# kernel-matrix-benchmarks/kernel-matrix-benchmarks

Measured on AMD Instinct MI355X. Metric: point-pair interactions/s (N*M/s) + max |err| vs scipy, D=3 Gaussian, higher is better.
Workload: dtype f32

## Files before the change

kernel_matrix_benchmarks_amd/csrc/kmvp_api.hip:

```cpp
#include "kmvp_ctx.hpp"

namespace kmvp {

Rccl g_rccl;

namespace {
thread_local std::string g_create_error;
}

int fail(kmvp_ctx* c, int code, const std::string& msg) {
  if (c) c->err = msg;
  else g_create_error = msg;
  return code;
}
const char* create_error() { return g_create_error.c_str(); }

int ensure(kmvp_ctx* c, DevBuf& b, size_t bytes) {
  if (bytes <= b.cap && b.p) return KMVP_OK;
  if (b.p) {
    HIP_TRY(c, hipFree(b.p));
    b.p = nullptr;
    b.cap = 0;
  }
  if (bytes == 0) bytes = 16;
// ... 284 lines not shown
    g_rccl.CommDestroy(c->comm);
    c->comm = nullptr;
  }
  c->host_xchg = fn;
  c->host_user = user;
  c->comm_count = world;
  c->rank = rank;
  c->world = world;
  return KMVP_OK;
}

int kmvp_comm_world(const kmvp_ctx* c) { return (c && c->exchanges()) ? c->comm_count : 1; }
int kmvp_comm_rank(const kmvp_ctx* c) { return (c && c->exchanges()) ? c->rank : 0; }

int kmvp_set_option(kmvp_ctx* c, const char* key, int64_t value) {
  if (!c || !key) return KMVP_E_INVALID;
  const std::string k(key);
  if (k == "feed") {
    if (value < -1 || value > 1) return fail(c, KMVP_E_INVALID, "feed must be -1 (auto), 0 or 1");
    c->opt_feed = (int)value;
  } else if (k == "targets_per_lane") {
    if (value != 0 && value != 1 && value != 2 && value != 4 && value != 8)
      return fail(c, KMVP_E_INVALID, "targets_per_lane must be 0 (auto), 1, 2, 4 or 8");
    c->opt_T = (int)value;
  } else if (k == "segments") {
    if (value < 0 || value > 65535) return fail(c, KMVP_E_INVALID, "segments out of range");
    c->opt_segments = (int)value;
  } else if (k == "fast_sqdists") {
    if (value < -1 || value > 4) return fail(c, KMVP_E_INVALID, "fast_sqdists must be -1 (auto), 0, 1, 2, 3 or 4");
    c->opt_fast = (int)value;
  } else if (k == "cellmm_shape") {
    if (value < -1 || value > 1) return fail(c, KMVP_E_INVALID, "cellmm_shape must be -1 (by size), 0 (32x32x16) or 1 (16x16x32)");
    c->opt_cellmm_shape = (int)value;
  } else if (k == "cell_fused") {
    if (value < -1 || value > 1) return fail(c, KMVP_E_INVALID, "cell_fused must be -1 (automatic), 0 (two launches) or 1 (one launch where it applies)");
    c->opt_cell_fused = (int)value;
  } else if (k == "mfma_variant") {
    if (value != -1 && value != 0 && value != 1 && value != 4 && value != 5)
      return fail(c, KMVP_E_INVALID, "mfma_variant must be -1 (by kernel), 0, 1, 4 or 5");
    c->opt_mfma_variant = (int)value;
  } else if (k == "same_points_global") {
    c->opt_same_global = value != 0;
  } else if (k == "partial_shard") {
    c->opt_partial = value != 0;
  } else if (k == "fast_tiles") {
    if (value != 0 && value != 1 && value != 2 && value != 4 && value != 8)
      return fail(c, KMVP_E_INVALID, "fast_tiles must be 0 (auto), 1, 2, 4 or 8");
    c->opt_fast_tiles = (int)value;
  } else if (k == "chunk") {
    if (value < 8 || value > (1 << 24)) return fail(c, KMVP_E_INVALID, "chunk out of range");
    c->opt_chunk = (int)value;
  } else {
    return fail(c, KMVP_E_INVALID, "unknown option " + k);
  }
  return KMVP_OK;
}

int64_t kmvp_device_bytes(const kmvp_ctx* c) {
  if (!c) return 0;
  size_t t = 0;
  for (const DevBuf* b : {&c->y_raw, &c->x_raw, &c->b_raw, &c->xs, &c->rec, &c->x_scaled,
                          &c->y_scaled, &c->part, &c->partd, &c->aux, &c->sortbuf, &c->perm, &c->sums, &c->out, &c->scratch, &c->sdiag, &c->xchg, &c->kexp, &c->kshift, &c->xchgk, &c->kflag,
                    &c->sk_xs_x, &c->sk_rec_y, &c->sk_xs_y, &c->sk_rec_x, &c->sk_state,
                          &c->cell_tperm, &c->cell_sperm, &c->cell_tgrp, &c->cell_sgrp, &c->cell_slot, &c->cell_tmeta, &c->cell_sums, &c->cell_skey, &c->cell_scentre, &c->cell_scale})
    t += b->cap;
  return (int64_t)t;
// ... 9 lines not shown
```

kernel_matrix_benchmarks_amd/csrc/kmvp_cellmm.hpp:

```cpp
#pragma once
#include <hip/hip_runtime.h>
#include <stdint.h>

#include "kmvp_cell.hpp"

namespace kmvp {

#ifndef CMM_BF16
#define CMM_BF16 0
#endif
#if CMM_BF16
typedef __bf16 cmm_half;
#else
typedef _Float16 cmm_half;
#endif
typedef cmm_half f16x8 __attribute__((ext_vector_type(8)));
typedef cmm_half f16x2 __attribute__((ext_vector_type(2)));

constexpr int CMM_STAGE_TILES = 12;
constexpr int CMM_STAGE_BYTES = 8192;
constexpr int CMM_E_OFF = 0;
constexpr int CMM_B_OFF = CMM_STAGE_TILES * CELL_TILE * 16;
constexpr int CMM_HDR_OFF = CMM_B_OFF + CMM_STAGE_TILES * CELL_TILE * 4;
static_assert(CMM_HDR_OFF + CMM_STAGE_TILES * 16 <= CMM_STAGE_BYTES, "stage image too small");
// ... 229 lines not shown
        acc[tt] = __builtin_amdgcn_mfma_f32_32x32x16_f16(ya, xb[tt], acc[tt], 0, 0, 0);
#endif
      }
    }
    if (s + 1 < s_end) commit(buf ^ 1);
    __syncthreads();
  }
  if (key_s >= 0) fold();

  const double inv = (double)a.scale[1];
#pragma unroll
  for (int tt = 0; tt < TT; ++tt)
    if (h == 0) a.part[(int64_t)seg * a.n_slots + (tile0 + tt - a.tile_base) * CELL_TILE + r] = outd[tt] * inv;
}


__device__ __forceinline__ float cellmm16_fold4(float a, float b, float c, float d) {
  const auto p = __builtin_amdgcn_permlane16_swap(__float_as_uint(a), __float_as_uint(b), false, false);
  const float w0 = __uint_as_float(p[0]) + __uint_as_float(p[1]);
  const auto q = __builtin_amdgcn_permlane16_swap(__float_as_uint(c), __float_as_uint(d), false, false);
  const float w1 = __uint_as_float(q[0]) + __uint_as_float(q[1]);
  const auto r = __builtin_amdgcn_permlane32_swap(__float_as_uint(w0), __float_as_uint(w1), false, false);
  return __uint_as_float(r[0]) + __uint_as_float(r[1]);
}
__device__ __forceinline__ float cellmm16_sources_sum(float v) {
  v += cellmm_dpp<0x111, 0xf>(v);
  v += cellmm_dpp<0x112, 0xf>(v);
  v += cellmm_dpp<0x114, 0xf>(v);
  v += cellmm_dpp<0x118, 0xf>(v);
  return __int_as_float(__builtin_amdgcn_readlane(__float_as_int(v), 15)) +
         __int_as_float(__builtin_amdgcn_readlane(__float_as_int(v), 47));
}

#ifndef CMM16_NOFOLD
#define CMM16_NOFOLD 0
#endif

template <int TT>
__device__ __forceinline__ void cellmm16_body(const CellmmArgs& a, int bid, unsigned char (*lds)[CMM_STAGE_BYTES]) {
  static_assert(!CMM_BF16, "f16 operands only");
  constexpr int SB = CMM_STAGE_BYTES;
  constexpr int PIECES = SB / (16 * BLOCK_THREADS);
  constexpr float LOG2E = 1.4426950408889634f;
  constexpr int HT = 2 * TT;
  constexpr int NG = (HT + 3) / 4;

  int tb, seg;
  block_to_work(bid, a.segments, a.tile_blocks, tb, seg);
  const int lane = threadIdx.x & 63;
  const int wave = threadIdx.x >> 6;
  const int cc = lane & 15;
  const int kg = lane >> 4;
  const int h = kg & 1;
  const int rs = 16 * (kg >> 1) + cc;
  const int64_t tile0 = a.tile_base + ((int64_t)tb * WAVES_PER_BLOCK + wave) * TT;

  float cT[3];
  f16x8 xb[HT];
#pragma unroll
  for (int u = 0; u < HT; ++u) {
    const f32x4 v = *reinterpret_cast<const f32x4*>(a.xd + ((tile0 + (u >> 1)) * CELL_TILE + 16 * (u & 1) + cc) * 4);
    xb[u] = cellmm_target_operand(v, h);
  }
  {
    const f32x4 m = *reinterpret_cast<const f32x4*>(a.tmeta + tile0 * 4);
#pragma unroll
    for (int c = 0; c < 3; ++c) cT[c] = __int_as_float(__builtin_amdgcn_readfirstlane(__float_as_int(m[c])));
  }
// ... 11 lines not shown
  }

  f32x4 acc[HT];
#pragma unroll
  for (int u = 0; u < HT; ++u)
#pragma unroll
    for (int k = 0; k < 4; ++k) acc[u][k] = 0.f;

  const int64_t s_begin = (int64_t)seg * a.seg_stages;
  int64_t s_end = s_begin + a.seg_stages;
  if (s_end > a.m_stages) s_end = a.m_stages;

  f32x4 pre[PIECES];
  auto fetch = [&](int64_t s) {
    const unsigned char* src = a.img + s * SB;
#pragma unroll
    for (int p = 0; p < PIECES; ++p)
      pre[p] = *reinterpret_cast<const f32x4*>(src + (p * BLOCK_THREADS + (int)threadIdx.x) * 16);
  };
  auto commit = [&](int buf) {
#pragma unroll
    for (int p = 0; p < PIECES; ++p)
      *reinterpret_cast<f32x4*>(&lds[buf][(p * BLOCK_THREADS + (int)threadIdx.x) * 16]) = pre[p];
  };
  if (s_begin < s_end) {
    fetch(s_begin);
    commit(0);
  }
  __syncthreads();

  int key_s = -2;
  float S0 = 0.f, S0c = 0.f;
  float D1[3] = {0.f, 0.f, 0.f};

  auto fold = [&]() {
#if CMM16_NOFOLD
    asm volatile("" ::"v"(S0), "v"(S0c));
#else
    const float s0 = cellmm16_sources_sum(S0) * CMM_TARGET_SCALE;
    float x[4 * NG];
#pragma unroll
    for (int u = 0; u < 4 * NG; ++u) x[u] = u < HT ? (acc[u][0] + acc[u][1]) + (acc[u][2] + acc[u][3]) : 0.f;
#pragma unroll
    for (int g = 0; g < NG; ++g) {
      const float v = cellmm16_fold4(x[4 * g], x[4 * g + 1], x[4 * g + 2], x[4 * g + 3]);
      outd[g] += (double)(U[g] * ((v - vprev[g]) + s0));
      vprev[g] = v;
    }
#endif
    S0 = 0.f;
    S0c = 0.f;
  };
  auto new_cell = [&](const f32x4 cs, int ks) {
    if (key_s >= 0) fold();
    key_s = ks;
#pragma unroll
    for (int c = 0; c < 3; ++c) D1[c] = (cT[c] - cs[c]) * LOG2E;
#if !CMM16_NOFOLD
#pragma unroll
    for (int g = 0; g < NG; ++g) {
      float s2 = 0.f;
#pragma unroll
      for (int c = 0; c < 3; ++c) {
        const float df = dl[g][c] + (cT[c] - cs[c]);
        s2 = fmaf(df, df, s2);
      }
      U[g] = kexp2(s2 * -LOG2E);
    }
#endif
  };

  for (int64_t s = s_begin; s < s_end; ++s) {
    const int buf = (int)((s - s_begin) & 1);
    if (s + 1 < s_end) fetch(s + 1);
    const unsigned char* base = &lds[buf][0];
    const unsigned char* p_ef = base + CMM_E_OFF + rs * 16;
    const unsigned char* p_b = base + CMM_B_OFF + rs * 4;
    const f32x4* hdr = reinterpret_cast<const f32x4*>(base + CMM_HDR_OFF);
    const int keys = lane < CMM_STAGE_TILES ? __float_as_int(hdr[lane < CMM_STAGE_TILES ? lane : 0][3]) : -1;
#pragma unroll 1
    for (int q = 0; q < CMM_STAGE_TILES; ++q) {
      const int ks = __builtin_amdgcn_readlane(keys, q);
      if (ks < 0) break;
      if (ks != key_s) new_cell(hdr[q], ks);
      const f32x4 ef = *reinterpret_cast<const f32x4*>(p_ef);
      const float bq = *reinterpret_cast<const float*>(p_b);
      p_ef += CELL_TILE * 16;
      p_b += CELL_TILE * 4;
      const float m0 = h ? ef[2] : ef[0];
      const float m1 = h ? ef[0] : ef[1];
      const float m2 = h ? ef[2] : 1.f;
      const f32x4 a14 = f32x4{m0, m1 * m2, m0 * m0, m1 * ef[1]};
      const float a5 = ef[1] * m2;
      const float arg = fmaf(ef[0], D1[0], fmaf(ef[1], D1[1], fmaf(ef[2], D1[2], ef[3])));
      const float wb = kexp2(arg) * bq;
      {
        const float yk = wb - S0c;
        const float tk = S0 + yk;
        S0c = (tk - S0) - yk;
        S0 = tk;
      }
      const float u1 = a14[0] * wb, u2 = a14[1] * wb;
      const f16x2 R0 = cellmm_pk(u1, u2);
      const float c1 = (float)R0[0], c2 = (float)R0[1];
      const f16x2 R1 = cellmm_pk(u1 - c1, u2 - c2);
      const f16x2 R3 = cellmm_pk(a14[2] * wb, a14[3] * wb);
      const f16x2 R2 = cellmm_pk(c1, a5 * wb);
      i32x4 yw;
      yw[0] = __builtin_bit_cast(int, R0);
      yw[1] = __builtin_bit_cast(int, R1);
      yw[2] = __builtin_bit_cast(int, R2);
      yw[3] = __builtin_bit_cast(int, R3);
      const f16x8 ya = __builtin_bit_cast(f16x8, yw);
#pragma unroll
      for (int u = 0; u < HT; ++u) acc[u] = __builtin_amdgcn_mfma_f32_16x16x32_f16(ya, xb[u], acc[u], 0, 0, 0);
    }
    if (s + 1 < s_end) commit(buf ^ 1);
    __syncthreads();
  }
  if (key_s >= 0) fold();
#if CMM16_NOFOLD
#pragma unroll
  for (int u = 0; u < HT; ++u) asm volatile("" ::"v"(acc[u][0]), "v"(acc[u][1]), "v"(acc[u][2]), "v"(acc[u][3]));
#endif

  const double inv = (double)a.scale[1];
#pragma unroll
  for (int g = 0; g < NG; ++g)
    if (4 * g + kg < HT)
      a.part[(int64_t)seg * a.n_slots + (tile0 + 2 * g + (kg >> 1) - a.tile_base) * CELL_TILE + 16 * h + cc] = outd[g] * inv;
}

template <int TT>
__global__ void __launch_bounds__(BLOCK_THREADS) __attribute__((amdgpu_waves_per_eu(TT >= 8 ? 2 : 1)))
cellmm16_kernel(const CellmmArgs a, const CellmmArgs rest, const int main_grid) {
  __shared__ __attribute__((aligned(16))) unsigned char lds[2][CMM_STAGE_BYTES];
  if constexpr (TT > CELL_REST_TT) {
    const FusedCellWork w = fused_cell_work((int64_t)blockIdx.x, (int64_t)main_grid);
    if (w.list) {
      cellmm16_body<CELL_REST_TT>(rest, (int)w.local, lds);
      return;
    }
  }
  cellmm16_body<TT>(a, (int)blockIdx.x, lds);
}

hipError_t launch_cellmm_gaussian(int TT, int shape, const CellmmArgs& args, dim3 grid, hipStream_t stream, const char** kernel_name);
hipError_t launch_cellmm16_fused(int TT, const CellmmArgs& main, const CellmmArgs& rest, int64_t main_grid, int64_t rest_grid,
                                 hipStream_t stream, const char** kernel_name);

}
```

kernel_matrix_benchmarks_amd/csrc/kmvp_cellmm_inst.hip:

```cpp
#include <stdlib.h>
#include "kmvp_internal.hpp"
#include "kmvp_cellmm.hpp"

namespace kmvp {

static size_t cmm_dbg_lds() {
  static const size_t v = getenv("KMVP_DBG_LDS") ? (size_t)atol(getenv("KMVP_DBG_LDS")) : 0;
  return v;
}
template <typename K, typename... Rest>
static void cmm_launch(K kernel, const CellmmArgs& args, dim3 grid, hipStream_t stream, Rest... rest) {
  if (cmm_dbg_lds()) (void)hipFuncSetAttribute((const void*)kernel, hipFuncAttributeMaxDynamicSharedMemorySize, (int)cmm_dbg_lds());
  hipLaunchKernelGGL(kernel, grid, dim3(BLOCK_THREADS), cmm_dbg_lds(), stream, args, rest...);
}

hipError_t launch_cellmm_gaussian(int TT, int shape, const CellmmArgs& args, dim3 grid, hipStream_t stream, const char** kernel_name) {
  if (kernel_name) *kernel_name = shape == 1 ? "cellmm16_kernel" : "cellmm_kernel";
  if (shape == 1) {
    const int all = (int)grid.x;
    switch (TT) {
      case 1: cmm_launch(cellmm16_kernel<1>, args, grid, stream, args, all); break;
      case 2: cmm_launch(cellmm16_kernel<2>, args, grid, stream, args, all); break;
      case 4: cmm_launch(cellmm16_kernel<4>, args, grid, stream, args, all); break;
      case 8: cmm_launch(cellmm16_kernel<8>, args, grid, stream, args, all); break;
      default: return hipErrorInvalidValue;
    }
    return hipGetLastError();
  }
  switch (TT) {
    case 1: cmm_launch(cellmm_kernel<1>, args, grid, stream); break;
    case 2: cmm_launch(cellmm_kernel<2>, args, grid, stream); break;
    case 4: cmm_launch(cellmm_kernel<4>, args, grid, stream); break;
    case 8: cmm_launch(cellmm_kernel<8>, args, grid, stream); break;
    default: return hipErrorInvalidValue;
  }
  return hipGetLastError();
}

hipError_t launch_cellmm16_fused(int TT, const CellmmArgs& main, const CellmmArgs& rest, int64_t main_grid, int64_t rest_grid,
                                 hipStream_t stream, const char** kernel_name) {
  if (kernel_name) *kernel_name = "cellmm16_kernel";
  if (main_grid + rest_grid > MAX_GRID) return hipErrorInvalidConfiguration;
  const dim3 grid((unsigned)(main_grid + rest_grid));
  switch (TT) {
    case 4: cmm_launch(cellmm16_kernel<4>, main, grid, stream, rest, (int)main_grid); break;
    case 8: cmm_launch(cellmm16_kernel<8>, main, grid, stream, rest, (int)main_grid); break;
    default: return hipErrorInvalidValue;
  }
  return hipGetLastError();
}

}
```

kernel_matrix_benchmarks_amd/csrc/kmvp_ctx.hpp:

```cpp
#pragma once
#include <dlfcn.h>
#include <hip/hip_runtime.h>
#include <rccl/rccl.h>
#include <stdint.h>
#include <stdlib.h>
#include <string.h>

#include <algorithm>
#include <cmath>
#include <string>
#include <vector>

#include "../../include/kmvp.h"
#include "kmvp_internal.hpp"

namespace kmvp {

enum : int { LAYOUT_LOWD = 0, LAYOUT_FAST = 1, LAYOUT_MFMA = 2, LAYOUT_CFAST = 3, LAYOUT_CELL = 4, LAYOUT_CELL64 = 5, LAYOUT_CELLMM = 6, LAYOUT_FASTMM = 7, LAYOUT_CFASTMM = 8 };

struct DevBuf {
  void* p = nullptr;
  size_t cap = 0;
};

// ... 70 lines not shown
  bool have_points = false, have_signal = false, density = false;
  bool async_product = false;
  bool diag_on = false;
  int64_t diag_n = 0;
  double diag_ridge = 0.0, diag_min = 0.0;

  DevBuf y_raw, x_raw, b_raw;
  DevBuf xs, rec;
  DevBuf partd;
  DevBuf aux;
  DevBuf sortbuf, perm;
  DevBuf x_scaled, y_scaled;
  DevBuf cell_tperm, cell_sperm, cell_tgrp, cell_sgrp, cell_slot, cell_tmeta, cell_sums, cell_skey, cell_scentre, cell_scale;
  DevBuf part, sums, out;
  DevBuf xchg;
  DevBuf kexp, kshift, xchgk;
  DevBuf kflag;
  DevBuf scratch;
  DevBuf sdiag;
  DevBuf sk_xs_x, sk_rec_y, sk_xs_y, sk_rec_x, sk_state;
  uint64_t sk_points_ver = 0;
  uint64_t points_ver = 0, signal_ver = 0;
  int packed_layout = -1;
  int packed_kernel = -1, packed_sig = -1, packed_T = -1;
  uint64_t packed_points_ver = 0, packed_signal_ver = 0;
  int gen_kernel = -1;
  uint64_t gen_points_ver = 0;
  int64_t out_n = 0;
  int out_e = 0;

  int opt_feed = -1, opt_T = 0, opt_segments = 0, opt_chunk = 512;
  int opt_fast = -1, opt_fast_tiles = 0;
  int opt_cellmm_shape = -1;
  int opt_cell_fused = -1;
  int opt_mfma_variant = -1;
  int opt_same_global = 0;
  int opt_partial = 0;
  uint64_t perm_ver = 0;
  uint64_t cell_ver = 0;
  int cell_state = 0;
  int cell_tt = 0, cell_tt_req = 0;
  float cell_lo[3] = {0.f, 0.f, 0.f}, cell_hh[3] = {1.f, 1.f, 1.f};
  int cell_g[3] = {1, 1, 1};
  int64_t cell_n_tiles = 0, cell_m_tiles = 0;
  int64_t cell_n_main = 0, cell_n_rest = 0;
  float cloud_radius2 = INFINITY;
  uint64_t centre_ver = 0;

  ncclComm_t comm = nullptr;
  int rank = 0, world = 1;
  kmvp_host_allreduce_fn host_xchg = nullptr;
  void* host_user = nullptr;
  std::vector<double> host_buf;
  bool exchanges() const { return comm != nullptr || host_xchg != nullptr; }

  int comm_count = 1;
  float last_kernel_ms = 0.f, last_total_ms = 0.f, last_allreduce_ms = 0.f;
  const char* last_kernel_name = "";
  std::string note;
};

namespace kmvp {

int fail(kmvp_ctx* c, int code, const std::string& msg);
const char* create_error();

#define HIP_TRY(c, expr)                                                                     \
  do {                                                                                       \
    hipError_t e_ = (expr);                                                                  \
    if (e_ != hipSuccess)                                                                    \
      return kmvp::fail((c), e_ == hipErrorOutOfMemory ? KMVP_E_NOMEM : KMVP_E_DEVICE,       \
                        std::string(#expr) + ": " + hipGetErrorString(e_));                  \
  } while (0)

inline size_t elem_size(int dtype) { return dtype == KMVP_F64 ? 8 : 4; }
inline unsigned blocks_for(int64_t n, int threads = 256) { return (unsigned)((n + threads - 1) / threads); }

// ... 20 lines not shown
```

kernel_matrix_benchmarks_amd/csrc/kmvp_internal.hpp:

```cpp
#pragma once
#include <hip/hip_runtime.h>
#include <stdint.h>

#include "kmvp_lowd.hpp"

namespace kmvp {

struct LowdTuning {
  int targets_per_lane;
  int feed;
};

constexpr int LOWD_MAX_D = 8;
constexpr int LOWD_MAX_E = 4;

constexpr int DEFAULT_TARGETS_PER_LANE = 1;
constexpr int DEFAULT_FEED = 1;

#define KMVP_DECLARE_LOWD(NAME, REAL)                                                           \
  hipError_t NAME(int D, int E, int sig, LowdTuning tune, const LowdArgs<REAL>& args, dim3 grid, \
                  hipStream_t stream, const char** kernel_name);                                \
  hipError_t NAME##_generic(int sig, const REAL* x, const REAL* y, const REAL* b, double* part,  \
                            int64_t n, int64_t n_pad, int64_t m, int D, int E, int NE,           \
                            int segments, int64_t seg_len, int64_t j_offset, int64_t m_total,    \
// ... 124 lines not shown
                               hipStream_t stream, const char** kernel_name);


constexpr double FMM_PS_PER_TILE_16 = 180.0, FMM_PS_PER_TILE_32 = 225.0;
constexpr double CMM_PS_PER_TILE_MAIN = 26.0, CMM_PS_PER_TILE_TT4 = 30.0, CMM_PS_PER_TILE_REST = 48.0;
struct FastmmArgs;
hipError_t launch_fastmm_gaussian(int KS, int mode, int TT, int online, const FastmmArgs& args, dim3 grid, hipStream_t stream,
                                  const char** kernel_name);
hipError_t launch_fastmm_absexp(int KS, int mode, int TT, int online, const FastmmArgs& args, dim3 grid, hipStream_t stream,
                                const char** kernel_name);
constexpr float FMM_ABSEXP_KAPPA = 5.0e-3f;

struct CfastmmArgs;
hipError_t launch_cfastmm(int kernel, int mode, int TT, int online, const CfastmmArgs& args, dim3 grid, hipStream_t stream,
                          const char** kernel_name);
constexpr int CFMM_AUTO_MIN_COLS = 4;

constexpr int CFAST_MAX_D = 4;
constexpr int CFAST_DEFAULT_TT = 2;
constexpr int LOWD_MID_MAX_D = 128;
struct CfastArgs;
hipError_t launch_cfast_gaussian(int sig, int TT, const CfastArgs& args, dim3 grid, hipStream_t stream,
                                 const char** kernel_name);
hipError_t launch_cfast_absexp(int sig, int TT, const CfastArgs& args, dim3 grid, hipStream_t stream,
                               const char** kernel_name);
hipError_t launch_cfast_invdist(int sig, int TT, const CfastArgs& args, dim3 grid, hipStream_t stream,
                                const char** kernel_name);
constexpr int CELL_MAX_D = 3;
constexpr double CELL_AUTO_MAX_PAD = 1.30;
struct CellArgs;
hipError_t launch_cell_gaussian(int sig, int TT, const CellArgs& args, dim3 grid, hipStream_t stream,
                                const char** kernel_name);
struct CellmmArgs;
hipError_t launch_cellmm_gaussian(int TT, int shape, const CellmmArgs& args, dim3 grid, hipStream_t stream, const char** kernel_name);
struct Cell64Args;
hipError_t launch_cell64_gaussian(int sig, const Cell64Args& args, dim3 grid, hipStream_t stream, const char** kernel_name);
hipError_t sort_pairs_u32(void* tmp, size_t* tmp_bytes, const unsigned* keys_in, unsigned* keys_out,
                          const int* vals_in, int* vals_out, int64_t n, hipStream_t stream);

}
```

kernel_matrix_benchmarks_amd/csrc/kmvp_plan.hpp:

```cpp
#pragma once
#include <algorithm>
#include <cstdint>
#include <vector>

namespace kmvp {

constexpr int WAVES_PER_BLOCK = 4;
constexpr int CELL_TILE = 32;
constexpr int CELL_REST_TT = 2;
constexpr int STAGED_TILE = 32;
constexpr int64_t SMALL_PROBLEM_TARGETS = 32768;
constexpr int SEG_SPLIT_FROM = 16;
constexpr int64_t MAX_GRID = 0x7fffffff;

inline int64_t round_up(int64_t v, int64_t q) { return (v + q - 1) / q * q; }
inline bool small_problem(int64_t N) { return N < SMALL_PROBLEM_TARGETS; }


struct SegmentRule {
  int64_t stage_bytes;
  int cols;
  int64_t min_seg = 1;
  bool small = false;
  int64_t l2_seg_bytes = 2 << 20;
// ... 106 lines not shown

struct CellTiles {
  int64_t main_live, main_empty, rest_live, rest_empty;
};
inline CellTiles split_cell_tiles(int64_t tiles, int TT) {
  const int64_t rem = tiles % TT;
  if (TT > CELL_REST_TT && rem > 0 && rem <= TT / 2) return {tiles - rem, 0, rem, round_up(rem, CELL_REST_TT) - rem};
  return {tiles, round_up(tiles, TT) - tiles, 0, 0};
}

inline void cell_split_count(const unsigned* keys, int64_t n, int TT, int64_t* n_main, int64_t* n_rest) {
  *n_main = *n_rest = 0;
  for_each_key_run(keys, n, [&](int64_t, int64_t cnt, unsigned) {
    const CellTiles s = split_cell_tiles((cnt + CELL_TILE - 1) / CELL_TILE, TT);
    *n_main += s.main_live + s.main_empty;
    *n_rest += s.rest_live + s.rest_empty;
  });
}

inline TileList cell_tiles_split(const unsigned* keys, int64_t n, int TT, int64_t* n_main, int64_t* n_rest) {
  TileList main, rest;
  main.reserve((size_t)n / 24 + 64);
  for_each_key_run(keys, n, [&](int64_t p, int64_t cnt, unsigned k) {
    const CellTiles s = split_cell_tiles((cnt + CELL_TILE - 1) / CELL_TILE, TT);
    main.add_cell(p, p, p + cnt, k, s.main_live, s.main_empty, CELL_TILE);
    rest.add_cell(p, p + s.main_live * CELL_TILE, p + cnt, k, s.rest_live, s.rest_empty, CELL_TILE);
  });
  main.pad_to((size_t)TT * WAVES_PER_BLOCK);
  rest.pad_to((size_t)CELL_REST_TT * WAVES_PER_BLOCK);
  *n_main = (int64_t)main.size();
  *n_rest = (int64_t)rest.size();
  main.append(rest);
  return main;
}

struct CellSplit {
  int64_t m_stages, n_slots;
  int64_t blocks[2], slots[2], seg_stages[2];
  int segments[2];
  int64_t grid(int r) const { return blocks[r] * segments[r]; }
  size_t region_offset(int cols, int r) const { return r ? (size_t)segments[0] * cols * slots[0] : 0; }
  size_t part_doubles(int cols) const { return ((size_t)segments[0] * slots[0] + (size_t)segments[1] * slots[1]) * cols; }
};

inline CellSplit cell_split(int64_t N, int64_t m_tiles, int64_t n_main, int64_t n_rest, int tt, int opt_segments,
                            int stage_tiles, SegmentRule main) {
  CellSplit s;
  main.small = small_problem(N);
  if (main.small) main.min_seg = 1;
  s.m_stages = (m_tiles + stage_tiles - 1) / stage_tiles;
  s.n_slots = (n_main + n_rest) * CELL_TILE;
  s.blocks[0] = n_main / (tt * WAVES_PER_BLOCK);
  s.blocks[1] = n_rest / (CELL_REST_TT * WAVES_PER_BLOCK);
  s.slots[0] = n_main * CELL_TILE;
  s.slots[1] = n_rest * CELL_TILE;
  s.segments[0] = stage_segments(opt_segments, std::max<int64_t>(1, s.blocks[0]), s.m_stages, s.n_slots, main);
  s.seg_stages[0] = (s.m_stages + s.segments[0] - 1) / s.segments[0];
  s.segments[1] = 0;
  s.seg_stages[1] = 1;
  if (s.blocks[1] > 0) {
    SegmentRule rest = main;
    rest.min_seg = 1;
    rest.target_blocks = 1536;
    const int seg = choose_segments(opt_segments, s.blocks[1], s.m_stages, s.n_slots, rest);
    s.seg_stages[1] = (s.m_stages + seg - 1) / seg;
    s.segments[1] = (int)((s.m_stages + s.seg_stages[1] - 1) / s.seg_stages[1]);
// ... 28 lines not shown
```

kernel_matrix_benchmarks_amd/csrc/kmvp_product.hip:

```cpp
#include "kmvp_ctx.hpp"
#include <vector>
#include "kmvp_cell_pack.hpp"
#include "kmvp_cell64_pack.hpp"
#include "kmvp_cellmm_pack.hpp"
#include "kmvp_cfast_pack.hpp"
#include "kmvp_fast_pack.hpp"
#include "kmvp_fastmm_pack.hpp"
#include "kmvp_cfastmm_pack.hpp"
#include "kmvp_mfma_pack.hpp"

namespace kmvp {
namespace {

template <typename real>
hipError_t launch_lowd(int kernel, int D, int E, int sig, LowdTuning tune,
                       const LowdArgs<real>& args, dim3 grid, hipStream_t s, const char** name);
template <>
hipError_t launch_lowd<float>(int kernel, int D, int E, int sig, LowdTuning tune,
                              const LowdArgs<float>& args, dim3 grid, hipStream_t s,
                              const char** name) {
  switch (kernel) {
    case K_GAUSSIAN: return launch_lowd_gaussian_f32(D, E, sig, tune, args, grid, s, name);
    case K_ABSEXP: return launch_lowd_absexp_f32(D, E, sig, tune, args, grid, s, name);
    case K_INVDIST: return launch_lowd_invdist_f32(D, E, sig, tune, args, grid, s, name);
// ... 1228 lines not shown
inline double cell_ps_per_tile(int TT) { return TT >= 8 ? CMM_PS_PER_TILE_MAIN : (TT >= 4 ? CMM_PS_PER_TILE_TT4 : CMM_PS_PER_TILE_REST); }

int cell_prepare(kmvp_ctx* c, int TT) {
  if (c->cell_ver == c->points_ver && c->cell_state != 0 && (c->cell_state < 0 || c->cell_tt_req == TT)) return KMVP_OK;
  c->cell_tt_req = TT;
  c->cell_ver = c->points_ver;
  c->cell_state = -1;
  const int D = c->D;
  if (D > CELL_MAX_D || !(c->cloud_radius2 < INFINITY) || c->N > 0x3fffffff || c->M > 0x3fffffff) return KMVP_OK;
  float aux[FAST_AUX_FLOATS];
  HIP_TRY(c, hipMemcpyAsync(aux, c->aux.p, sizeof(aux), hipMemcpyDeviceToHost, c->stream));
  HIP_TRY(c, hipStreamSynchronize(c->stream));
  CellGrid grid;
  if (!cell_make_grid(aux, D, (float)(std::sqrt(2.f * CELL_T_MAX / (float)D)), grid)) return KMVP_OK;
  int rc;
  std::vector<unsigned> keys;
  if ((rc = cell_sort(c, c->y_raw.p, c->M, grid, c->cell_sperm, keys))) return rc;
  const TileList sources = cell_tiles(keys.data(), c->M);
  if ((rc = upload_tiles(c, sources, c->cell_sgrp))) return rc;
  c->cell_m_tiles = (int64_t)sources.size();
  if (!c->same_points && (rc = cell_sort(c, c->x_raw.p, c->N, grid, c->cell_tperm, keys))) return rc;
  if (TT == 0) {
    double best = INFINITY;
    for (int t : {8, 4, 2}) {
      int64_t nm, nr;
      cell_split_count(keys.data(), (int64_t)keys.size(), t, &nm, &nr);
      const double cost = cell_ps_per_tile(t) * (double)nm + cell_ps_per_tile(2) * (double)nr;
      if (cost < best) {
        best = cost;
        TT = t;
      }
    }
  }
  if ((rc = upload_tiles(c, cell_tiles_split(keys.data(), (int64_t)keys.size(), TT, &c->cell_n_main, &c->cell_n_rest), c->cell_tgrp)))
    return rc;
  c->cell_n_tiles = c->cell_n_main + c->cell_n_rest;
  c->cell_tt = TT;
  cell_store_grid(c, grid);
  c->cell_state = 1;
  c->packed_layout = -1;
  return KMVP_OK;
}

double cell_padding(const kmvp_ctx* c) {
  const double t = (double)c->cell_n_tiles * CELL_TILE / (double)std::max<int64_t>(c->N, 1);
  const double s = (double)c->cell_m_tiles * CELL_TILE / (double)std::max<int64_t>(c->M, 1);
  return std::max(t, s);
}

CellSplit cell_plan(const kmvp_ctx* c, int stage_tiles, SegmentRule main) {
  return cell_split(c->N, c->cell_m_tiles, c->cell_n_main, c->cell_n_rest, c->cell_tt, c->opt_segments, stage_tiles, main);
}
double* cell_region(const kmvp_ctx* c, const CellSplit& s, int cols, int r) { return (double*)c->part.p + s.region_offset(cols, r); }
template <class Args>
void cell_args(const kmvp_ctx* c, const CellSplit& s, int cols, int r, Args& a) {
  a.part = cell_region(c, s, cols, r);
  a.n_slots = s.slots[r];
  a.tile_base = r ? c->cell_n_main : 0;
  a.seg_stages = s.seg_stages[r];
  a.segments = s.segments[r];
  a.tile_blocks = (int)s.blocks[r];
}
inline int cell_tt(const kmvp_ctx* c, int r) { return r ? CELL_REST_TT : c->cell_tt; }

int pack_cell_targets(kmvp_ctx* c, const CellGrid& grid) {
  const int64_t n_tiles = c->cell_n_tiles;
  const float* x_raw = (const float*)(c->same_points ? c->y_raw.p : c->x_raw.p);
  const int* tperm = (const int*)(c->same_points ? c->cell_sperm.p : c->cell_tperm.p);
// ... 85 lines not shown
  rule.min_seg = 2;
  rule.l2_seg_bytes = 3 << 20;
  rule.target_blocks = 7168;
  const CellSplit s = cell_plan(c, CMM_STAGE_TILES, rule);
  const int64_t m_stages = s.m_stages, n_slots = s.n_slots;
  int rc;
  CellGrid grid;
  cell_load_grid(c, grid);

  const PackKey key = {LAYOUT_CELLMM, K_GAUSSIAN, TT};
  const int image_sig = NE > 1 ? -1 : sig;
  const bool sig_stale = signal_stale(c, key, image_sig);
  const int* sgrp = (const int*)c->cell_sgrp.p;
  if ((rc = ensure(c, c->cell_scale, 64))) return rc;
  float* scale = (float*)c->cell_scale.p;
  unsigned* bmax = (unsigned*)c->cell_scale.p + 4;
  HIP_TRY(c, mark(c, 0));
  if (points_stale(c, key)) {
    if ((rc = pack_cell_targets(c, grid))) return rc;
    if ((rc = ensure(c, c->rec, (size_t)m_stages * CMM_STAGE_BYTES))) return rc;
    hipLaunchKernelGGL(pack_cellmm_points_kernel, dim3((unsigned)(m_stages * CMM_STAGE_TILES)), dim3(CELL_TILE), 0,
                       c->stream, (const float*)c->y_raw.p, (const int*)c->cell_sperm.p, sgrp, sgrp + c->cell_m_tiles,
                       (const unsigned*)(sgrp + 2 * c->cell_m_tiles), c->cell_m_tiles, D, grid, (unsigned char*)c->rec.p);
    HIP_TRY(c, hipGetLastError());
  }
  record_packed(c, key, image_sig);

  if ((rc = ensure(c, c->part, s.part_doubles(1) * sizeof(double)))) return rc;
  if ((rc = ensure(c, c->sums, (size_t)NE * N * sizeof(double)))) return rc;
  if ((rc = ensure(c, c->cell_sums, (size_t)NE * n_slots * sizeof(double)))) return rc;
  const int shape = c->opt_cellmm_shape >= 0 ? c->opt_cellmm_shape : ((TT >= 8 && c->N >= 500000 && c->M >= 100000) ? 1 : 0);
  FusedCellGrid fg = fused_cell_grid(s, TT, c->opt_cell_fused);
  if (shape != 1) fg.fused = false;
  CellmmArgs a;
  a.xd = (const float*)c->xs.p;
  a.tmeta = (const float*)c->cell_tmeta.p;
  a.img = (const unsigned char*)c->rec.p;
  a.scale = scale;
  a.m_stages = m_stages;
  if (NE == 1 && !sig_stale) HIP_TRY(c, mark(c, 0));
  for (int col = 0; col < NE; ++col) {
    if (sig_stale) {
      const float* b = (sig == SIG_DENSITY || col == E) ? (const float*)nullptr : (const float*)c->b_raw.p;
      HIP_TRY(c, hipMemsetAsync(bmax, 0, sizeof(unsigned), c->stream));
      if (b)
        hipLaunchKernelGGL(cellmm_absmax_kernel, dim3((unsigned)std::min<int64_t>(1024, (c->M + 255) / 256)), dim3(256), 0,
                           c->stream, b, c->M, E, col, bmax);
      hipLaunchKernelGGL(cellmm_scale_kernel, dim3(1), dim3(1), 0, c->stream, (const unsigned*)bmax, cellmm_wlog2(c),
                         b ? 0 : 1, scale);
      hipLaunchKernelGGL(pack_cellmm_signal_kernel, dim3((unsigned)(m_stages * CMM_STAGE_TILES)), dim3(CELL_TILE), 0,
                         c->stream, b, E, col, (const int*)c->cell_sperm.p, sgrp, sgrp + c->cell_m_tiles, c->cell_m_tiles,
                         (const float*)scale, (unsigned char*)c->rec.p);
      HIP_TRY(c, hipGetLastError());
      if (NE == 1) HIP_TRY(c, mark(c, 0));
    }
    hipError_t le = hipSuccess;
    if (fg.fused) {
      CellmmArgs ar = a;
      cell_args(c, s, 1, 0, a);
      cell_args(c, s, 1, 1, ar);
      le = launch_cellmm16_fused(TT, a, ar, fg.main_grid, fg.rest_grid, c->stream, &c->last_kernel_name);
    } else {
      for (int r = 0; r < 2 && le == hipSuccess; ++r)
        if (s.blocks[r] > 0) {
          cell_args(c, s, 1, r, a);
          le = launch_cellmm_gaussian(cell_tt(c, r), shape, a, dim3((unsigned)s.grid(r)), c->stream, &c->last_kernel_name);
        }
    }
    if (le == hipErrorInvalidValue) return fail(c, KMVP_E_UNSUPPORTED, "fast_tiles must be 1, 2, 4 or 8");
    HIP_TRY(c, le);
    if (NE == 1) HIP_TRY(c, mark(c, 1));
    double* col_sums = (double*)c->cell_sums.p + (size_t)col * n_slots;
    for (int r = 0; r < 2; ++r)
      if (s.blocks[r] > 0)
        hipLaunchKernelGGL(reduce_segments_kernel, dim3(blocks_for(s.slots[r])), dim3(256), 0, c->stream,
                           (const double*)cell_region(c, s, 1, r), col_sums + (r ? s.slots[0] : 0), s.slots[r], s.segments[r], 0);
    HIP_TRY(c, hipGetLastError());
  }
  if (NE > 1) HIP_TRY(c, mark(c, 1));

  hipLaunchKernelGGL(gather_cells_kernel, dim3(blocks_for((int64_t)NE * N)), dim3(256), 0, c->stream,
                     (const double*)c->cell_sums.p, (const int*)c->cell_slot.p, (double*)c->sums.p, N, n_slots, NE);
  HIP_TRY(c, hipGetLastError());
  return finish_product(c, (int64_t)NE * N, N, N, E, sig);
}


int cell64_prepare(kmvp_ctx* c) {
  if (c->cell_ver == c->points_ver && c->cell_state != 0) return KMVP_OK;
  c->cell_ver = c->points_ver;
  c->cell_state = -1;
  const int D = c->D;
  if (D > CELL_MAX_D || !(c->cloud_radius2 < INFINITY) || c->N > 0x3fffffff || c->M > 0x3fffffff) return KMVP_OK;
  float aux[FAST_AUX_FLOATS];
  HIP_TRY(c, hipMemcpyAsync(aux, c->aux.p, sizeof(aux), hipMemcpyDeviceToHost, c->stream));
  HIP_TRY(c, hipStreamSynchronize(c->stream));
  CellGrid grid;
  if (!cell_make_grid(aux, D, (float)((float)std::sqrt(2.0 * CELL64_T_MAX / (double)D)), grid)) return KMVP_OK;
  int rc;
// ... 592 lines not shown
```

Measured before the change: 42690 billion.

## Build cellmm16 source operands once per workgroup in LDS when tiles share a cell

Adds a shared-build variant of the 16x16x32 cell MFMA kernel. When every MAIN workgroup's target tiles lie in one cell, each wave builds a quarter of the stage's source operands (exp weights and f16 split operands) and writes them to LDS. All waves then read the prebuilt operands instead of each recomputing exp and the packing per tile. This cuts redundant VALU/transcendental work by roughly the wave count. The cost is a larger LDS footprint, extra LDS traffic, and a host-side uniformity check that decides eligibility.

```diff
diff --git a/kernel_matrix_benchmarks_amd/csrc/kmvp_api.hip b/kernel_matrix_benchmarks_amd/csrc/kmvp_api.hip
--- a/kernel_matrix_benchmarks_amd/csrc/kmvp_api.hip
+++ b/kernel_matrix_benchmarks_amd/csrc/kmvp_api.hip
@@ -340,6 +340,9 @@
   } else if (k == "cellmm_shape") {
     if (value < -1 || value > 1) return fail(c, KMVP_E_INVALID, "cellmm_shape must be -1 (by size), 0 (32x32x16) or 1 (16x16x32)");
     c->opt_cellmm_shape = (int)value;
+  } else if (k == "cell_shared") {
+    if (value < -1 || value > 1) return fail(c, KMVP_E_INVALID, "cell_shared must be -1 (automatic), 0 (never) or 1 (where every MAIN workgroup lies in one cell)");
+    c->opt_cell_shared = (int)value;
   } else if (k == "cell_fused") {
     if (value < -1 || value > 1) return fail(c, KMVP_E_INVALID, "cell_fused must be -1 (automatic), 0 (two launches) or 1 (one launch where it applies)");
     c->opt_cell_fused = (int)value;
diff --git a/kernel_matrix_benchmarks_amd/csrc/kmvp_cellmm.hpp b/kernel_matrix_benchmarks_amd/csrc/kmvp_cellmm.hpp
--- a/kernel_matrix_benchmarks_amd/csrc/kmvp_cellmm.hpp
+++ b/kernel_matrix_benchmarks_amd/csrc/kmvp_cellmm.hpp
@@ -285,8 +285,34 @@
          __int_as_float(__builtin_amdgcn_readlane(__float_as_int(v), 47));
 }
 
+__device__ __forceinline__ i32x4 cellmm16_source_operand(const f32x4 ef, const float bq, const float (&D1)[3], const int h, float& w) {
+  const float m0 = h ? ef[2] : ef[0];
+  const float m1 = h ? ef[0] : ef[1];
+  const float m2 = h ? ef[2] : 1.f;
+  const f32x4 a14 = f32x4{m0, m1 * m2, m0 * m0, m1 * ef[1]};
+  const float a5 = ef[1] * m2;
+  const float arg = fmaf(ef[0], D1[0], fmaf(ef[1], D1[1], fmaf(ef[2], D1[2], ef[3])));
+  w = kexp2(arg);
+  const float wb = w * bq;
+  const float u1 = a14[0] * wb, u2 = a14[1] * wb;
+  const f16x2 R0 = cellmm_pk(u1, u2);
+  const float c1 = (float)R0[0], c2 = (float)R0[1];
+  const f16x2 R1 = cellmm_pk(fmaf(a14[0], wb, -c1), fmaf(a14[1], wb, -c2));
+  const f16x2 R3 = cellmm_pk(a14[2] * wb, a14[3] * wb);
+  const f16x2 R2 = cellmm_pk(c1, a5 * wb);
+  i32x4 yw;
+  yw[0] = __builtin_bit_cast(int, R0);
+  yw[1] = __builtin_bit_cast(int, R1);
+  yw[2] = __builtin_bit_cast(int, R2);
+  yw[3] = __builtin_bit_cast(int, R3);
+  return yw;
+}
+
 #ifndef CMM16_NOFOLD
 #define CMM16_NOFOLD 0
+#endif
+#ifndef CMM16_QUARTER_BUILD
+#define CMM16_QUARTER_BUILD 0
 #endif
 
 template <int TT>
@@ -364,6 +390,10 @@
   int key_s = -2;
   float S0 = 0.f, S0c = 0.f;
   float D1[3] = {0.f, 0.f, 0.f};
+#if CMM16_QUARTER_BUILD
+  i32x4 ykeep = {0, 0, 0, 0};
+  const int wave_u = __builtin_amdgcn_readfirstlane(wave);
+#endif
 
   auto fold = [&]() {
 #if CMM16_NOFOLD
@@ -419,31 +449,31 @@
       const float bq = *reinterpret_cast<const float*>(p_b);
       p_ef += CELL_TILE * 16;
       p_b += CELL_TILE * 4;
-      const float m0 = h ? ef[2] : ef[0];
-      const float m1 = h ? ef[0] : ef[1];
-      const float m2 = h ? ef[2] : 1.f;
-      const f32x4 a14 = f32x4{m0, m1 * m2, m0 * m0, m1 * ef[1]};
-      const float a5 = ef[1] * m2;
-      const float arg = fmaf(ef[0], D1[0], fmaf(ef[1], D1[1], fmaf(ef[2], D1[2], ef[3])));
-      const float wb = kexp2(arg) * bq;
-      {
-        const float yk = wb - S0c;
+#if CMM16_QUARTER_BUILD
+      if (TT == 8 && (q & 3) != wave_u) {
+        asm volatile("" ::"v"(ef[0]), "v"(ef[1]), "v"(ef[2]), "v"(ef[3]));
+        const float yk = bq - S0c;
         const float tk = S0 + yk;
         S0c = (tk - S0) - yk;
         S0 = tk;
-      }
-      const float u1 = a14[0] * wb, u2 = a14[1] * wb;
-      const f16x2 R0 = cellmm_pk(u1, u2);
-      const float c1 = (float)R0[0], c2 = (float)R0[1];
-      const f16x2 R1 = cellmm_pk(u1 - c1, u2 - c2);
-      const f16x2 R3 = cellmm_pk(a14[2] * wb, a14[3] * wb);
-      const f16x2 R2 = cellmm_pk(c1, a5 * wb);
-      i32x4 yw;
-      yw[0] = __builtin_bit_cast(int, R0);
-      yw[1] = __builtin_bit_cast(int, R1);
-      yw[2] = __builtin_bit_cast(int, R2);
-      yw[3] = __builtin_bit_cast(int, R3);
+        asm volatile("" : "+v"(ykeep[0]), "+v"(ykeep[1]), "+v"(ykeep[2]), "+v"(ykeep[3]));
+      } else {
+#endif
+      float w;
+      const i32x4 yw = cellmm16_source_operand(ef, bq, D1, h, w);
+      {
+        const float yk = fmaf(bq, w, -S0c);
+        const float tk = S0 + yk;
+        S0c = (tk - S0) - yk;
+        S0 = tk;
+      }
+#if CMM16_QUARTER_BUILD
+      ykeep = yw;
+      }
+      const f16x8 ya = __builtin_bit_cast(f16x8, ykeep);
+#else
       const f16x8 ya = __builtin_bit_cast(f16x8, yw);
+#endif
 #pragma unroll
       for (int u = 0; u < HT; ++u) acc[u] = __builtin_amdgcn_mfma_f32_16x16x32_f16(ya, xb[u], acc[u], 0, 0, 0);
     }
@@ -463,10 +493,179 @@
       a.part[(int64_t)seg * a.n_slots + (tile0 + 2 * g + (kg >> 1) - a.tile_base) * CELL_TILE + 16 * h + cc] = outd[g] * inv;
 }
 
+constexpr int CMS_YA_OFF = 0;
+constexpr int CMS_WB_OFF = CMM_STAGE_TILES * 64 * 16;
+constexpr int CMS_HDR_OFF = CMS_WB_OFF + CMM_STAGE_TILES * CELL_TILE * 8;
+constexpr int CMS_STAGE_BYTES = CMS_HDR_OFF + CMM_STAGE_TILES * 16;
+constexpr int CMS_BUILD_TILES = CMM_STAGE_TILES / WAVES_PER_BLOCK;
+static_assert(CMS_BUILD_TILES * WAVES_PER_BLOCK == CMM_STAGE_TILES, "every tile of a stage has one builder");
+
 template <int TT>
+__device__ __forceinline__ void cellmm16_shared_body(const CellmmArgs& a, int bid, unsigned char* lds) {
+  static_assert(!CMM_BF16, "f16 operands only");
+  constexpr int SB = CMM_STAGE_BYTES;
+  constexpr float LOG2E = 1.4426950408889634f;
+  constexpr int HT = 2 * TT;
+  constexpr int NG = (HT + 3) / 4;
+  constexpr int NB = CMS_BUILD_TILES;
+
+  int tb, seg;
+  block_to_work(bid, a.segments, a.tile_blocks, tb, seg);
+  const int lane = threadIdx.x & 63;
+  const int wave = __builtin_amdgcn_readfirstlane(threadIdx.x >> 6);
+  const int cc = lane & 15;
+  const int kg = lane >> 4;
+  const int h = kg & 1;
+  const int rs = 16 * (kg >> 1) + cc;
+  const int64_t tile0 = a.tile_base + ((int64_t)tb * WAVES_PER_BLOCK + wave) * TT;
+
+  float cT[3];
+  f16x8 xb[HT];
+#pragma unroll
+  for (int u = 0; u < HT; ++u) {
+    const f32x4 v = *reinterpret_cast<const f32x4*>(a.xd + ((tile0 + (u >> 1)) * CELL_TILE + 16 * (u & 1) + cc) * 4);
+    xb[u] = cellmm_target_operand(v, h);
+  }
+  {
+    const f32x4 m = *reinterpret_cast<const f32x4*>(a.tmeta + tile0 * 4);
+#pragma unroll
+    for (int c = 0; c < 3; ++c) cT[c] = __int_as_float(__builtin_amdgcn_readfirstlane(__float_as_int(m[c])));
+  }
+  float dl[NG][3], U[NG], vprev[NG];
+  double outd[NG];
+#pragma unroll
+  for (int g = 0; g < NG; ++g) {
+    const int u = 4 * g + kg < HT ? 4 * g + kg : HT - 1;
+    const f32x4 v = *reinterpret_cast<const f32x4*>(a.xd + ((tile0 + (u >> 1)) * CELL_TILE + 16 * (u & 1) + cc) * 4);
+#pragma unroll
+    for (int c = 0; c < 3; ++c) dl[g][c] = v[c];
+    U[g] = 0.f;
+    vprev[g] = 0.f;
+    outd[g] = 0.0;
+  }
+
+  f32x4 acc[HT];
+#pragma unroll
+  for (int u = 0; u < HT; ++u)
+#pragma unroll
+    for (int k = 0; k < 4; ++k) acc[u][k] = 0.f;
+
+  const int64_t s_begin = (int64_t)seg * a.seg_stages;
+  int64_t s_end = s_begin + a.seg_stages;
+  if (s_end > a.m_stages) s_end = a.m_stages;
+
+  f32x4 pe[NB], ph[NB];
+  float pb[NB];
+  auto fetch = [&](int64_t s) {
+    const unsigned char* src = a.img + s * SB;
+#pragma unroll
+    for (int j = 0; j < NB; ++j) {
+      const int t = NB * wave + j;
+      pe[j] = *reinterpret_cast<const f32x4*>(src + CMM_E_OFF + (t * CELL_TILE + rs) * 16);
+      pb[j] = *reinterpret_cast<const float*>(src + CMM_B_OFF + (t * CELL_TILE + rs) * 4);
+      ph[j] = *reinterpret_cast<const f32x4*>(src + CMM_HDR_OFF + t * 16);
+    }
+  };
+  auto build = [&](int buf) {
+    unsigned char* base = lds + buf * CMS_STAGE_BYTES;
+#pragma unroll
+    for (int j = 0; j < NB; ++j) {
+      const int t = NB * wave + j;
+      if (lane == 0) *reinterpret_cast<f32x4*>(base + CMS_HDR_OFF + t * 16) = ph[j];
+      if (__builtin_amdgcn_readfirstlane(__float_as_int(ph[j][3])) < 0) continue;
+      float D1[3], w;
+#pragma unroll
+      for (int c = 0; c < 3; ++c) D1[c] = (cT[c] - ph[j][c]) * LOG2E;
+      const i32x4 yw = cellmm16_source_operand(pe[j], pb[j], D1, h, w);
+      *reinterpret_cast<i32x4*>(base + CMS_YA_OFF + (t * 64 + lane) * 16) = yw;
+      if (h == 0) *reinterpret_cast<f32x2*>(base + CMS_WB_OFF + (t * CELL_TILE + rs) * 8) = f32x2{w, pb[j]};
+    }
+  };
+  if (s_begin < s_end) {
+    fetch(s_begin);
+    build(0);
+  }
+  __syncthreads();
+
+  int key_s = -2;
+  float S0 = 0.f, S0c = 0.f;
+
+  auto fold = [&]() {
+    const float s0 = cellmm16_sources_sum(S0) * CMM_TARGET_SCALE;
+    float x[4 * NG];
+#pragma unroll
+    for (int u = 0; u < 4 * NG; ++u) x[u] = u < HT ? (acc[u][0] + acc[u][1]) + (acc[u][2] + acc[u][3]) : 0.f;
+#pragma unroll
+    for (int g = 0; g < NG; ++g) {
+      const float v = cellmm16_fold4(x[4 * g], x[4 * g + 1], x[4 * g + 2], x[4 * g + 3]);
+      outd[g] += (double)(U[g] * ((v - vprev[g]) + s0));
+      vprev[g] = v;
+    }
+    S0 = 0.f;
+    S0c = 0.f;
+  };
+  auto new_cell = [&](const f32x4 cs, int ks) {
+    if (key_s >= 0) fold();
+    key_s = ks;
+#pragma unroll
+    for (int g = 0; g < NG; ++g) {
+      float s2 = 0.f;
+#pragma unroll
+      for (int c = 0; c < 3; ++c) {
+        const float df = dl[g][c] + (cT[c] - cs[c]);
+        s2 = fmaf(df, df, s2);
+      }
+      U[g] = kexp2(s2 * -LOG2E);
+    }
+  };
+
+  for (int64_t s = s_begin; s < s_end; ++s) {
+    const int buf = (int)((s - s_begin) & 1);
+    const bool more = s + 1 < s_end;
+    if (more) fetch(s + 1);
+    const unsigned char* base = lds + buf * CMS_STAGE_BYTES;
+    const unsigned char* p_ya = base + CMS_YA_OFF + lane * 16;
+    const unsigned char* p_wb = base + CMS_WB_OFF + rs * 8;
+    const f32x4* hdr = reinterpret_cast<const f32x4*>(base + CMS_HDR_OFF);
+    const int keys = lane < CMM_STAGE_TILES ? __float_as_int(hdr[lane < CMM_STAGE_TILES ? lane : 0][3]) : -1;
+#pragma unroll 1
+    for (int q = 0; q < CMM_STAGE_TILES; ++q) {
+      const int ks = __builtin_amdgcn_readlane(keys, q);
+      if (ks < 0) break;
+      if (ks != key_s) new_cell(hdr[q], ks);
+      const i32x4 yw = *reinterpret_cast<const i32x4*>(p_ya);
+      const f32x2 wq = *reinterpret_cast<const f32x2*>(p_wb);
+      p_ya += 64 * 16;
+      p_wb += CELL_TILE * 8;
+      {
+        const float yk = fmaf(wq[1], wq[0], -S0c);
+        const float tk = S0 + yk;
+        S0c = (tk - S0) - yk;
+        S0 = tk;
+      }
+      const f16x8 ya = __builtin_bit_cast(f16x8, yw);
+#pragma unroll
+      for (int u = 0; u < HT; ++u) acc[u] = __builtin_amdgcn_mfma_f32_16x16x32_f16(ya, xb[u], acc[u], 0, 0, 0);
+    }
+    if (more) build(buf ^ 1);
+    __syncthreads();
+  }
+  if (key_s >= 0) fold();
+
+  const double inv = (double)a.scale[1];
+#pragma unroll
+  for (int g = 0; g < NG; ++g)
+    if (4 * g + kg < HT)
+      a.part[(int64_t)seg * a.n_slots + (tile0 + 2 * g + (kg >> 1) - a.tile_base) * CELL_TILE + 16 * h + cc] = outd[g] * inv;
+}
+
+template <int TT, bool SHARED = false>
 __global__ void __launch_bounds__(BLOCK_THREADS) __attribute__((amdgpu_waves_per_eu(TT >= 8 ? 2 : 1)))
 cellmm16_kernel(const CellmmArgs a, const CellmmArgs rest, const int main_grid) {
-  __shared__ __attribute__((aligned(16))) unsigned char lds[2][CMM_STAGE_BYTES];
+  static_assert(!SHARED || TT > CELL_REST_TT, "the shared-build body exists for TT = 8 and 4");
+  constexpr int LDS_BYTES = 2 * (SHARED ? CMS_STAGE_BYTES : CMM_STAGE_BYTES);
+  __shared__ __attribute__((aligned(16))) unsigned char lds_bytes[LDS_BYTES];
+  unsigned char(*lds)[CMM_STAGE_BYTES] = reinterpret_cast<unsigned char(*)[CMM_STAGE_BYTES]>(lds_bytes);
   if constexpr (TT > CELL_REST_TT) {
     const FusedCellWork w = fused_cell_work((int64_t)blockIdx.x, (int64_t)main_grid);
     if (w.list) {
@@ -474,11 +673,15 @@
       return;
     }
   }
-  cellmm16_body<TT>(a, (int)blockIdx.x, lds);
-}
-
-hipError_t launch_cellmm_gaussian(int TT, int shape, const CellmmArgs& args, dim3 grid, hipStream_t stream, const char** kernel_name);
+  if constexpr (SHARED)
+    cellmm16_shared_body<TT>(a, (int)blockIdx.x, lds_bytes);
+  else
+    cellmm16_body<TT>(a, (int)blockIdx.x, lds);
+}
+
+hipError_t launch_cellmm_gaussian(int TT, int shape, const CellmmArgs& args, dim3 grid, hipStream_t stream, const char** kernel_name,
+                                  bool shared);
 hipError_t launch_cellmm16_fused(int TT, const CellmmArgs& main, const CellmmArgs& rest, int64_t main_grid, int64_t rest_grid,
-                                 hipStream_t stream, const char** kernel_name);
-
-}
+                                 bool shared, hipStream_t stream, const char** kernel_name);
+
+}
diff --git a/kernel_matrix_benchmarks_amd/csrc/kmvp_cellmm_inst.hip b/kernel_matrix_benchmarks_amd/csrc/kmvp_cellmm_inst.hip
--- a/kernel_matrix_benchmarks_amd/csrc/kmvp_cellmm_inst.hip
+++ b/kernel_matrix_benchmarks_amd/csrc/kmvp_cellmm_inst.hip
@@ -14,15 +14,16 @@
   hipLaunchKernelGGL(kernel, grid, dim3(BLOCK_THREADS), cmm_dbg_lds(), stream, args, rest...);
 }
 
-hipError_t launch_cellmm_gaussian(int TT, int shape, const CellmmArgs& args, dim3 grid, hipStream_t stream, const char** kernel_name) {
+hipError_t launch_cellmm_gaussian(int TT, int shape, const CellmmArgs& args, dim3 grid, hipStream_t stream, const char** kernel_name,
+                                  bool shared) {
   if (kernel_name) *kernel_name = shape == 1 ? "cellmm16_kernel" : "cellmm_kernel";
   if (shape == 1) {
     const int all = (int)grid.x;
     switch (TT) {
       case 1: cmm_launch(cellmm16_kernel<1>, args, grid, stream, args, all); break;
       case 2: cmm_launch(cellmm16_kernel<2>, args, grid, stream, args, all); break;
-      case 4: cmm_launch(cellmm16_kernel<4>, args, grid, stream, args, all); break;
-      case 8: cmm_launch(cellmm16_kernel<8>, args, grid, stream, args, all); break;
+      case 4: shared ? cmm_launch(cellmm16_kernel<4, true>, args, grid, stream, args, all) : cmm_launch(cellmm16_kernel<4>, args, grid, stream, args, all); break;
+      case 8: shared ? cmm_launch(cellmm16_kernel<8, true>, args, grid, stream, args, all) : cmm_launch(cellmm16_kernel<8>, args, grid, stream, args, all); break;
       default: return hipErrorInvalidValue;
     }
     return hipGetLastError();
@@ -38,13 +39,13 @@
 }
 
 hipError_t launch_cellmm16_fused(int TT, const CellmmArgs& main, const CellmmArgs& rest, int64_t main_grid, int64_t rest_grid,
-                                 hipStream_t stream, const char** kernel_name) {
+                                 bool shared, hipStream_t stream, const char** kernel_name) {
   if (kernel_name) *kernel_name = "cellmm16_kernel";
   if (main_grid + rest_grid > MAX_GRID) return hipErrorInvalidConfiguration;
   const dim3 grid((unsigned)(main_grid + rest_grid));
   switch (TT) {
-    case 4: cmm_launch(cellmm16_kernel<4>, main, grid, stream, rest, (int)main_grid); break;
-    case 8: cmm_launch(cellmm16_kernel<8>, main, grid, stream, rest, (int)main_grid); break;
+    case 4: shared ? cmm_launch(cellmm16_kernel<4, true>, main, grid, stream, rest, (int)main_grid) : cmm_launch(cellmm16_kernel<4>, main, grid, stream, rest, (int)main_grid); break;
+    case 8: shared ? cmm_launch(cellmm16_kernel<8, true>, main, grid, stream, rest, (int)main_grid) : cmm_launch(cellmm16_kernel<8>, main, grid, stream, rest, (int)main_grid); break;
     default: return hipErrorInvalidValue;
   }
   return hipGetLastError();
diff --git a/kernel_matrix_benchmarks_amd/csrc/kmvp_ctx.hpp b/kernel_matrix_benchmarks_amd/csrc/kmvp_ctx.hpp
--- a/kernel_matrix_benchmarks_amd/csrc/kmvp_ctx.hpp
+++ b/kernel_matrix_benchmarks_amd/csrc/kmvp_ctx.hpp
@@ -126,6 +126,7 @@
   int opt_feed = -1, opt_T = 0, opt_segments = 0, opt_chunk = 512;
   int opt_fast = -1, opt_fast_tiles = 0;
   int opt_cellmm_shape = -1;
+  int opt_cell_shared = -1;
   int opt_cell_fused = -1;
   int opt_mfma_variant = -1;
   int opt_same_global = 0;
@@ -137,6 +138,7 @@
   float cell_lo[3] = {0.f, 0.f, 0.f}, cell_hh[3] = {1.f, 1.f, 1.f};
   int cell_g[3] = {1, 1, 1};
   int64_t cell_n_tiles = 0, cell_m_tiles = 0;
+  bool cell_main_uniform = false;
   int64_t cell_n_main = 0, cell_n_rest = 0;
   float cloud_radius2 = INFINITY;
   uint64_t centre_ver = 0;
diff --git a/kernel_matrix_benchmarks_amd/csrc/kmvp_internal.hpp b/kernel_matrix_benchmarks_amd/csrc/kmvp_internal.hpp
--- a/kernel_matrix_benchmarks_amd/csrc/kmvp_internal.hpp
+++ b/kernel_matrix_benchmarks_amd/csrc/kmvp_internal.hpp
@@ -180,7 +180,8 @@
 hipError_t launch_cell_gaussian(int sig, int TT, const CellArgs& args, dim3 grid, hipStream_t stream,
                                 const char** kernel_name);
 struct CellmmArgs;
-hipError_t launch_cellmm_gaussian(int TT, int shape, const CellmmArgs& args, dim3 grid, hipStream_t stream, const char** kernel_name);
+hipError_t launch_cellmm_gaussian(int TT, int shape, const CellmmArgs& args, dim3 grid, hipStream_t stream, const char** kernel_name,
+                                  bool shared);
 struct Cell64Args;
 hipError_t launch_cell64_gaussian(int sig, const Cell64Args& args, dim3 grid, hipStream_t stream, const char** kernel_name);
 hipError_t sort_pairs_u32(void* tmp, size_t* tmp_bytes, const unsigned* keys_in, unsigned* keys_out,
diff --git a/kernel_matrix_benchmarks_amd/csrc/kmvp_plan.hpp b/kernel_matrix_benchmarks_amd/csrc/kmvp_plan.hpp
--- a/kernel_matrix_benchmarks_amd/csrc/kmvp_plan.hpp
+++ b/kernel_matrix_benchmarks_amd/csrc/kmvp_plan.hpp
@@ -162,6 +162,15 @@
   *n_rest = (int64_t)rest.size();
   main.append(rest);
   return main;
+}
+
+inline bool main_list_cell_uniform(const unsigned* keys, int64_t n_main, int tt) {
+  const int64_t group = (int64_t)tt * WAVES_PER_BLOCK;
+  if (n_main % group) return false;
+  for (int64_t g = 0; g < n_main; g += group)
+    for (int64_t t = 1; t < group; ++t)
+      if (keys[g + t] != keys[g]) return false;
+  return true;
 }
 
 struct CellSplit {
diff --git a/kernel_matrix_benchmarks_amd/csrc/kmvp_product.hip b/kernel_matrix_benchmarks_amd/csrc/kmvp_product.hip
--- a/kernel_matrix_benchmarks_amd/csrc/kmvp_product.hip
+++ b/kernel_matrix_benchmarks_amd/csrc/kmvp_product.hip
@@ -1284,8 +1284,9 @@
       }
     }
   }
-  if ((rc = upload_tiles(c, cell_tiles_split(keys.data(), (int64_t)keys.size(), TT, &c->cell_n_main, &c->cell_n_rest), c->cell_tgrp)))
-    return rc;
+  const TileList targets = cell_tiles_split(keys.data(), (int64_t)keys.size(), TT, &c->cell_n_main, &c->cell_n_rest);
+  c->cell_main_uniform = main_list_cell_uniform(targets.key.data(), c->cell_n_main, TT);
+  if ((rc = upload_tiles(c, targets, c->cell_tgrp))) return rc;
   c->cell_n_tiles = c->cell_n_main + c->cell_n_rest;
   c->cell_tt = TT;
   cell_store_grid(c, grid);
@@ -1437,6 +1438,16 @@
   const int shape = c->opt_cellmm_shape >= 0 ? c->opt_cellmm_shape : ((TT >= 8 && c->N >= 500000 && c->M >= 100000) ? 1 : 0);
   FusedCellGrid fg = fused_cell_grid(s, TT, c->opt_cell_fused);
   if (shape != 1) fg.fused = false;
+  bool shared = false;
+  if (shape == 1 && s.blocks[0] > 0) {
+    const char* why = c->opt_cell_shared == 0 ? "cell_shared = 0"
+                      : TT <= CELL_REST_TT    ? "fewer than four target tiles per wavefront"
+                      : !c->cell_main_uniform ? "a MAIN workgroup's target tiles span more than one cell"
+                                              : nullptr;
+    shared = why == nullptr;
+    c->note = shared ? "cellmm16_kernel: shared-build body (each source operand built once per workgroup)"
+                     : std::string("cellmm16_kernel: per-wave build (") + why + ")";
+  }
   CellmmArgs a;
   a.xd = (const float*)c->xs.p;
   a.tmeta = (const float*)c->cell_tmeta.p;
@@ -1464,12 +1475,13 @@
       CellmmArgs ar = a;
       cell_args(c, s, 1, 0, a);
       cell_args(c, s, 1, 1, ar);
-      le = launch_cellmm16_fused(TT, a, ar, fg.main_grid, fg.rest_grid, c->stream, &c->last_kernel_name);
+      le = launch_cellmm16_fused(TT, a, ar, fg.main_grid, fg.rest_grid, shared, c->stream, &c->last_kernel_name);
     } else {
       for (int r = 0; r < 2 && le == hipSuccess; ++r)
         if (s.blocks[r] > 0) {
           cell_args(c, s, 1, r, a);
-          le = launch_cellmm_gaussian(cell_tt(c, r), shape, a, dim3((unsigned)s.grid(r)), c->stream, &c->last_kernel_name);
+          le = launch_cellmm_gaussian(cell_tt(c, r), shape, a, dim3((unsigned)s.grid(r)), c->stream, &c->last_kernel_name,
+                                         r == 0 && shared);
         }
     }
     if (le == hipErrorInvalidValue) return fail(c, KMVP_E_UNSUPPORTED, "fast_tiles must be 1, 2, 4 or 8");
```

After: 43140 billion (median of 6 runs). 1.01x the previous value.
